# noorgme/Decentralised-Verification-and-Distributed-Execution-of-Large-Scale-Video-Diffusion-Models

Measured on AMD Instinct MI355X. Metric: denoising steps/sec, Zeroscope-XL 24f@1024x576 (CFG UNet3D forward + guidance + DDIM), higher is better.
Workload: dtype f16

## Files before the change

### decentralised-verification-and-distributed-execution-of-large-scale-video-diffusion-models_amd/_lib.py

```python
from __future__ import annotations

import ctypes as C
import os

_HERE = os.path.dirname(os.path.abspath(__file__))
LIB_PATH = os.environ.get("VDX_LIB_PATH") or os.path.join(_HERE, "libvdx_hip.so")


class GemmArgs(C.Structure):
    _fields_ = [
        ("a", C.c_void_p), ("a2", C.c_void_p), ("w", C.c_void_p), ("bias", C.c_void_p),
        ("bias2", C.c_void_p), ("residual", C.c_void_p), ("out", C.c_void_p),
        ("M", C.c_int32), ("N", C.c_int32), ("K", C.c_int32), ("mode", C.c_int32),
        ("c1", C.c_int32), ("c2", C.c_int32),
        ("lda", C.c_int32), ("lda2", C.c_int32), ("ldo", C.c_int32), ("ldr", C.c_int32),
        ("h_in", C.c_int32), ("w_in", C.c_int32), ("h_out", C.c_int32), ("w_out", C.c_int32),
        ("stride", C.c_int32), ("upsample", C.c_int32), ("frames", C.c_int32), ("hw", C.c_int32),
        ("rows_per_bias2", C.c_int32), ("ldb2", C.c_int32), ("epilogue", C.c_int32),
        ("row_begin", C.c_int32), ("row_end", C.c_int32),
        ("ksplit", C.c_int32), ("wset_rows", C.c_int32), ("workspace", C.c_void_p), ("wset_bias", C.c_void_p),
        ("workspace_bytes", C.c_size_t), ("pad_mode", C.c_int32),
    ]


class ClipPreprocessArgs(C.Structure):
    _fields_ = [
        ("frames", C.c_void_p), ("x_bounds", C.c_void_p), ("x_coeffs", C.c_void_p), ("y_bounds", C.c_void_p),
        ("y_coeffs", C.c_void_p), ("out", C.c_void_p), ("out_u8", C.c_void_p),
        ("frame_pitch", C.c_size_t), ("row_pitch", C.c_int32), ("F", C.c_int32), ("H", C.c_int32), ("W", C.c_int32),
        ("kx", C.c_int32), ("ky", C.c_int32), ("band", C.c_int32), ("span", C.c_int32), ("ldo", C.c_int32),
    ]


_vp, _i, _f, _sz = C.c_void_p, C.c_int, C.c_float, C.c_size_t

SIGNATURES = {
    "vdx_last_error": (C.c_char_p, []),
    "vdx_version": (_i, []),
    "vdx_build_flags": (_i, []),
    "vdx_gemm_f16": (_i, [C.POINTER(GemmArgs), _vp]),
    "vdx_gemm_plan": (_i, [C.POINTER(GemmArgs), C.POINTER(C.c_int32), C.POINTER(C.c_int32)]),
    "vdx_gemm_kernel_name": (_i, [C.POINTER(GemmArgs), C.c_char_p, _sz]),
    "vdx_gemm_plan_ksplit": (_i, [C.POINTER(GemmArgs), C.POINTER(C.c_int32), C.POINTER(C.c_int32), C.POINTER(C.c_size_t)]),
    "vdx_softmax_rows_f16": (_i, [_vp, _i, _i, _i, _f, _vp]),
    "vdx_rows_to_u8_frames": (_i, [_vp, _i, _sz, _vp, _vp]),
    "vdx_im2col_in_f16": (_i, [_vp, _vp, _i, _i, _i, _i, _i, _i, _vp]),
    "vdx_rows_to_ncfhw_f16": (_i, [_vp, _i, _vp, _i, _i, _i, _i, _i, _vp]),
    "vdx_silu_f16": (_i, [_vp, _vp, _sz, _vp]),
    "vdx_groupnorm_workspace": (_sz, [_i, _i, _i, _i]),
    "vdx_groupnorm_f16": (_i, [_vp, _i, _i, _vp, _i, _i, _vp, _vp, _f, _i, _i, _i, _i, _vp, _i, _vp, _vp]),
    "vdx_groupnorm_workspace_part": (_sz, [_i, _i, _i, _i, _i]),
    "vdx_groupnorm_part_f16": (_i, [_vp, _i, _i, _vp, _i, _i, _vp, _vp, _f, _i, _i, _i, _i, _vp, _i, _vp, _i, _vp]),
    "vdx_groupnorm_fold_linear_f16": (_i, [_vp, _i, _i, _vp, _vp, _f, _i, _i, _i, _vp, _i, _vp, _vp, _i, _vp, _vp, _vp]),
    "vdx_groupnorm_stats_f16": (_i, [_vp, _i, _i, _vp, _i, _i, _vp, _vp, _f, _i, _i, _i, _vp, _i, C.POINTER(_sz), _vp]),
    "vdx_conv3x3_gn_supported": (_i, [_i, _i, _i]),
    "vdx_conv3x3_gn_preferred": (_i, [_i, _i, _i, _i, _i, _i]),
    "vdx_conv3x3_gn_f16": (_i, [_vp, _i, _vp, _i, _i, _i, _vp, _vp, _vp, _vp, _i, _i, _vp, _i, _vp, _i, _i, _i, _i, _i, _vp]),
    "vdx_tconv_gn_supported": (_i, [_i, _i, _i]),
    "vdx_tconv_gn_preferred": (_i, [_i, _i, _i, _i, _i]),
    "vdx_tconv_gn_f16": (_i, [_vp, _i, _vp, _vp, _vp, _vp, _i, _vp, _i, _i, _i, _i, _i, _i, _vp]),
    "vdx_layernorm_f16": (_i, [_vp, _i, _vp, _vp, _f, _i, _i, _vp, _i, _vp]),
    "vdx_flash_attn_f16": (_i, [_vp, _i, _vp, _i, _vp, _i, _vp, _i, _i, _i, _i, _i, _i, _i, _f, _i, _vp]),
    "vdx_flash_attn_rows_f16": (_i, [_vp, _i, _vp, _i, _vp, _i, _vp, _i, _i, _i, _i, _i, _i, _i, _f, _i, _vp]),
    "vdx_timestep_embedding_f16": (_i, [_vp, _vp, _i, _i, _vp]),
    "vdx_gelu_f16": (_i, [_vp, _vp, _sz, _vp]),
    "vdx_temporal_attn_f16": (_i, [_vp, _i, _vp, _i, _i, _i, _i, _i, _f, _vp]),
    "vdx_ff_block_supported": (_i, [_i]),
    "vdx_ff_block_pack_bytes": (_sz, [_i]),
    "vdx_ff_block_f16": (_i, [_vp, _i, _vp, _f, _vp, _i, _i, _i, _vp]),
    "vdx_ff_block_proj_pack_bytes": (_sz, [_i]),
    "vdx_ff_block_proj_f16": (_i, [_vp, _i, _vp, _f, _vp, _i, _i, _vp, _vp, _i, _i, _i, _vp]),
    "vdx_cross_attn_block_supported": (_i, [_i, _i]),
    "vdx_cross_attn_block_pack_bytes": (_sz, [_i]),
    "vdx_cross_attn_block_kv_bytes": (_sz, [_i]),
    "vdx_cross_attn_block_f16": (_i, [_vp, _i, _vp, _vp, _i, _f, _vp, _i, _i, _i, _i, _vp]),
    "vdx_temporal_attn_block_supported": (_i, [_i, _i]),
    "vdx_temporal_attn_block_wqkv_bytes": (_sz, [_i]),
    "vdx_temporal_attn_block_wo_bytes": (_sz, [_i]),
    "vdx_temporal_attn_block_f16": (_i, [_vp, _i, _vp, _vp, _f, _vp, _vp, _vp, _vp, _i, _i, _i, _i, _i, _f, _vp]),
    "vdx_temporal_attn_block2_supported": (_i, [_i, _i]),
    "vdx_temporal_attn_block2_pack_bytes": (_sz, [_i]),
    "vdx_temporal_attn_block2_f16": (_i, [_vp, _i, _vp, _f, _vp, _i, _i, _i, _i, _i, _vp]),
    "vdx_comm_unique_id": (_i, [_vp]),
    "vdx_comm_init": (_i, [_vp, _i, _i, C.POINTER(_vp)]),
    "vdx_comm_destroy": (_i, [_vp]),
    "vdx_allgather_shard": (_i, [_vp, _vp, _vp, _sz, _vp]),
    "vdx_halo_exchange": (_i, [_vp, _vp, _sz, _i, _vp, _sz, _i, _vp]),
    "vdx_ipc_export": (_i, [_vp, _vp, C.POINTER(_sz)]),
    "vdx_ipc_open": (_i, [_vp, _sz, C.POINTER(_vp)]),
    "vdx_ipc_close": (_i, [_vp, _sz]),
# ... 84 lines not shown
```

### decentralised-verification-and-distributed-execution-of-large-scale-video-diffusion-models_amd/ops.py

```python
from __future__ import annotations

import contextlib
import ctypes as C
from typing import Optional

import torch

from . import _lib
from ._lib import GemmArgs, VdxError

PLAIN, CONV3X3, TCONV3 = 0, 1, 2
EPI_GEGLU = 1


def _stream() -> int:
    return torch.cuda.current_stream().cuda_stream


def _p(t: Optional[torch.Tensor], name: str, dtype=torch.float16) -> Optional[int]:
    if t is None:
        return None
    if not t.is_cuda:
        raise VdxError(f"{name}: expected a GPU tensor (the denoising path has no CPU fallback)")
    if t.dtype != dtype:
# ... 423 lines not shown
def conv3x3_gn(x, gamma, beta, w, *, x2=None, bias=None, bias2=None, rows_per_bias2=0, residual=None, groups, n_img, h, wd, eps,
               partition_samples=0, out=None):
    r, c1, ldx = _rows(x, "x")
    S = h * wd
    M = n_img * S
    c2 = ldx2 = 0
    if x2 is not None:
        r2, c2, ldx2 = _rows(x2, "x2")
        if r2 < M:
            raise VdxError(f"conv3x3_gn: x2 has {r2} rows, need {M}")
    Cc = c1 + c2
    N, K = w.shape
    if r < M or K != 9 * Cc or gamma.numel() != Cc or beta.numel() != Cc or not w.is_contiguous():
        raise VdxError(f"conv3x3_gn: x [{r}][{c1}] (+{c2}), w [{N}][{K}], gamma {gamma.numel()}, M = {M}: shapes do not match")
    if not conv3x3_gn_supported(c1, c2, N):
        raise VdxError(f"conv3x3_gn: c1={c1}, c2={c2}, N={N} not supported")
    if bias is not None and bias.numel() != N:
        raise VdxError(f"conv3x3_gn: bias has {bias.numel()} elements, N={N}")
    ldb2 = _covers(bias2, M, N, "conv3x3_gn", "bias2", rows_per_bias2)
    ldr = _covers(residual, M, N, "conv3x3_gn", "residual")
    out, ldo = _out(out, M, N, x, "conv3x3_gn")
    need = _lib.load().vdx_groupnorm_workspace_part(n_img, S, Cc, groups, partition_samples)
    ws = _scratch(_GN_WS, x.device, need, torch.uint8, 1 << 20)
    off = C.c_size_t(0)
    _launch("vdx_groupnorm_stats_f16", _p(x, "x"), c1, ldx, _p(x2, "x2"), c2, ldx2, _p(gamma, "gamma"), _p(beta, "beta"),
            float(eps), groups, n_img, S, ws.data_ptr(), partition_samples, C.byref(off))
    with _timed("conv3x3_gn_kernel", 2.0 * M * N * K, (M, N, K)):
        _launch("vdx_conv3x3_gn_f16", _p(x, "x"), ldx, _p(x2, "x2"), ldx2, c1, c2, ws.data_ptr() + off.value, _p(w, "w"),
                _p(bias, "bias"), _p(bias2, "bias2"), rows_per_bias2, ldb2, _p(residual, "residual"), ldr, _p(out, "out"), ldo,
                n_img, h, wd, N)
    return out


def tconv_gn_supported(C: int, N: int, F: int) -> bool:
    return bool(_lib.load().vdx_tconv_gn_supported(C, N, F))


def tconv_gn_preferred(C: int, N: int, B: int, F: int, S: int) -> bool:
    return bool(_lib.load().vdx_tconv_gn_preferred(C, N, B, F, S))


def tconv_gn(x, gamma, beta, w, *, bias=None, residual=None, groups, B, F, S, eps, partition_samples=0, out=None):
    r, Cc, ldx = _rows(x, "x")
    M = B * F * S
    N, K = w.shape
    if r < M or K != 3 * Cc or gamma.numel() != Cc or beta.numel() != Cc or not w.is_contiguous():
        raise VdxError(f"tconv_gn: x [{r}][{Cc}], w [{N}][{K}], gamma {gamma.numel()}, M = {M}: shapes do not match")
    if not tconv_gn_supported(Cc, N, F):
        raise VdxError(f"tconv_gn: C={Cc}, N={N}, F={F} not supported")
    if bias is not None and bias.numel() != N:
        raise VdxError(f"tconv_gn: bias has {bias.numel()} elements, N={N}")
    ldr = _covers(residual, M, N, "tconv_gn", "residual")
    out, ldo = _out(out, M, N, x, "tconv_gn")
    need = _lib.load().vdx_groupnorm_workspace_part(B, F * S, Cc, groups, partition_samples)
    ws = _scratch(_GN_WS, x.device, need, torch.uint8, 1 << 20)
    off = C.c_size_t(0)
    _launch("vdx_groupnorm_stats_f16", _p(x, "x"), Cc, ldx, None, 0, 0, _p(gamma, "gamma"), _p(beta, "beta"), float(eps), groups, B,
            F * S, ws.data_ptr(), partition_samples, C.byref(off))
    with _timed(f"tconv_gn_kernel<{16 if F % 16 == 0 else 12 if F % 12 == 0 else 8}>", 2.0 * M * N * K, (M, N, K)):
        _launch("vdx_tconv_gn_f16", _p(x, "x"), ldx, ws.data_ptr() + off.value, _p(w, "w"), _p(bias, "bias"),
                _p(residual, "residual"), ldr, _p(out, "out"), ldo, B, F, S, Cc, N)
    return out


def layernorm(x, gamma, beta, *, M, eps=1e-5, out=None):
    r, Cc, ldx = _rows(x, "x")
# ... 511 lines not shown
```

### decentralised-verification-and-distributed-execution-of-large-scale-video-diffusion-models_amd/unet3d.py

```python
from __future__ import annotations

import math
import os
from dataclasses import dataclass
from types import SimpleNamespace
from typing import Dict, List, Optional, Tuple

import torch
import torch.nn as nn

from . import ops, packing
from ._lib import VdxError


@dataclass
class UNet3DConfig:
    in_channels: int = 4
    out_channels: int = 4
    block_out_channels: Tuple[int, ...] = (320, 640, 1280, 1280)
    layers_per_block: int = 2
    attention_head_dim: int = 64
    cross_attention_dim: int = 1024
    norm_num_groups: int = 32
    norm_eps: float = 1e-5
# ... 9 lines not shown


TEXT_PAD = 128


class UNet3DConditionModel(nn.Module):

    def __init__(self, cfg: Optional[UNet3DConfig] = None):
        super().__init__()
        self.cfg = cfg or UNet3DConfig.zeroscope()
        c = self.cfg
        if c.attention_head_dim != 64:
            raise VdxError("attention kernels are built for head_dim 64")
        for ch in c.block_out_channels:
            if ch % 64 != 0:
                raise VdxError("block_out_channels must be multiples of 64")
        if c.cross_attention_dim % 64 != 0:
            raise VdxError("cross_attention_dim must be a multiple of 64")
        self.config = SimpleNamespace(in_channels=c.in_channels, out_channels=c.out_channels,
                                      cross_attention_dim=c.cross_attention_dim,
                                      block_out_channels=c.block_out_channels,
                                      sample_size=None)
        self.W: Dict[str, torch.Tensor] = {}
        self._temb_slices: Dict[str, Tuple[int, int]] = {}
        self._device = torch.device("cpu")
        self.dtype = torch.float16
        self.ff_block_bytes = None
        self.lean_concat = True
        self.lean_attn = True
        self.fold_norm_proj_in = True
        self.fuse_ff = True
        self.fuse_cross_attn = True
        self.fuse_proj_out = True
        self.fuse_conv_gn = True
        self.fuse_tconv = True
        self.spatial_v_rows = True
        self.fuse_temporal_attention = True
        self.share_cfg_prefix = True
        self.detect_cfg_duplicate = False
        self._text_ref = None
        self._text_kv: Dict[str, tuple] = {}

    def _resnet_names(self) -> List[str]:
        c = self.cfg
        names = []
        for i, t in enumerate(c.down_block_types):
            names += [f"down_blocks.{i}.resnets.{j}" for j in range(c.layers_per_block)]
        names += ["mid_block.resnets.0", "mid_block.resnets.1"]
        for i, t in enumerate(c.up_block_types):
            names += [f"up_blocks.{i}.resnets.{j}" for j in range(c.layers_per_block + 1)]
        return names

    @torch.no_grad()
    def load_diffusers_state_dict(self, sd: Dict[str, torch.Tensor], device=None):
        dev = torch.device(device) if device is not None else self._device
        W: Dict[str, torch.Tensor] = {}

        def put(name, t):
            W[name] = t.to(device=dev, dtype=torch.float16).contiguous()

        used = set()

        def get(k):
            used.add(k)
            if k not in sd:
                raise VdxError(f"missing key in state dict: {k}")
# ... 496 lines not shown
        x = self._temp_conv("mid_block.temp_convs.0", x, B, F, hh * ww)
        x = self._spatial_transformer("mid_block.attentions.0", x, ehs_pad, n_img, F, hh, ww)
        x = self._temporal_transformer("mid_block.temp_attentions.0", x, B, F, hh * ww, x.shape[1] // 64)
        x = self._resnet("mid_block.resnets.1", x, None, temb_all, n_img, F, hh, ww)
        x = self._temp_conv("mid_block.temp_convs.1", x, B, F, hh * ww)
        for i, t in enumerate(c.up_block_types):
            p = f"up_blocks.{i}"
            for j in range(c.layers_per_block + 1):
                skip, sh, sw = skips.pop()
                if (sh, sw) != (hh, ww):
                    raise VdxError("skip connection resolution mismatch")
                if shared_skip and not skips:
                    skip = torch.cat([skip, skip])
                owned = [x, skip]
                x = skip = None
                x = self._resnet(f"{p}.resnets.{j}", owned, None, temb_all, n_img, F, hh, ww)
                x = self._temp_conv(f"{p}.temp_convs.{j}", x, B, F, hh * ww)
                if t.startswith("CrossAttn"):
                    x = self._spatial_transformer(f"{p}.attentions.{j}", x, ehs_pad, n_img, F, hh, ww)
                    x = self._temporal_transformer(f"{p}.temp_attentions.{j}", x, B, F, hh * ww, x.shape[1] // 64)
            if i != nlev - 1:
                th, tw = skips[-1][1], skips[-1][2]
                w_up = W[f"{p}.upsamplers.0.conv.weight"]
                if (th, tw) == (2 * hh, 2 * ww):
                    mode_up = 3
                elif hh <= th <= 2 * hh and ww <= tw <= 2 * ww:
                    mode_up = 2
                    w_up = W[f"{p}.upsamplers.0.conv.weight_taps9"]
                else:
                    raise VdxError(f"upsampler {p}: {hh}x{ww} -> {th}x{tw}")
                x = ops.gemm(x, w_up, M=n_img * th * tw, mode=ops.CONV3X3,
                             bias=W[f"{p}.upsamplers.0.conv.bias"], conv=(n_img, hh, ww, th, tw, 1, mode_up), allow_ksplit=True)
                hh, ww = th, tw
        n = ops.groupnorm(x, W["conv_norm_out.weight"], W["conv_norm_out.bias"], groups=c.norm_num_groups,
                          n_samples=n_img, rows_per_sample=hh * ww, eps=c.norm_eps, silu_act=True)
        y = ops.gemm(n, W["conv_out.weight"], M=n_img * hh * ww, mode=ops.CONV3X3, bias=W["conv_out.bias"],
                     conv=(n_img, hh, ww, hh, ww, 1, False))
        out = ops.rows_to_ncfhw(y, B, c.out_channels, F, hh, ww)
        return SimpleNamespace(sample=out)
```

### include/vdx.h

```cpp
#ifndef VDX_H
#define VDX_H
#include <stddef.h>
#include <stdint.h>

#ifdef __cplusplus
extern "C" {
#endif

typedef void* vdx_stream_t;

const char* vdx_last_error(void);
int vdx_version(void);
int vdx_build_flags(void);

enum { VDX_GEMM_PLAIN = 0, VDX_GEMM_CONV3X3 = 1, VDX_GEMM_TCONV3 = 2 };
enum { VDX_EPI_GEGLU = 1 };

typedef struct vdx_gemm_args {
    const void* a;
    const void* a2;
    const void* w;
    const void* bias;
    const void* bias2;
    const void* residual;
// ... 28 lines not shown
                      int Kpad, vdx_stream_t stream);

int vdx_rows_to_ncfhw_f16(const void* rows, int ld, void* out, int B, int C, int F, int H, int W,
                          vdx_stream_t stream);

int vdx_silu_f16(const void* x, void* y, size_t n, vdx_stream_t stream);

int vdx_timestep_embedding_f16(const float* t_device, void* out, int B, int dim, vdx_stream_t stream);

int vdx_gelu_f16(const void* x, void* y, size_t n, vdx_stream_t stream);

size_t vdx_groupnorm_workspace(int n_samples, int rows_per_sample, int C, int G);
int vdx_groupnorm_f16(const void* x, int c1, int ldx, const void* x2, int c2, int ldx2,
                      const void* gamma, const void* beta, float eps, int G,
                      int n_samples, int rows_per_sample, int silu,
                      void* y, int ldy, void* workspace, vdx_stream_t stream);
size_t vdx_groupnorm_workspace_part(int n_samples, int rows_per_sample, int C, int G, int partition_samples);
int vdx_groupnorm_fold_linear_f16(const void* x, int C, int ldx, const void* gamma, const void* beta, float eps, int G,
                                  int n_samples, int rows_per_sample, void* workspace, int partition_samples,
                                  const void* w, const void* bias, int N, void* w_out, void* bias_out, vdx_stream_t stream);
int vdx_groupnorm_part_f16(const void* x, int c1, int ldx, const void* x2, int c2, int ldx2,
                           const void* gamma, const void* beta, float eps, int G,
                           int n_samples, int rows_per_sample, int silu,
                           void* y, int ldy, void* workspace, int partition_samples, vdx_stream_t stream);
int vdx_groupnorm_stats_f16(const void* x, int c1, int ldx, const void* x2, int c2, int ldx2, const void* gamma,
                            const void* beta, float eps, int G, int n_samples, int rows_per_sample, void* workspace,
                            int partition_samples, size_t* scale_shift_offset, vdx_stream_t stream);
int vdx_conv3x3_gn_supported(int c1, int c2, int N);
int vdx_conv3x3_gn_preferred(int c1, int c2, int N, int n_img, int h, int w);
int vdx_conv3x3_gn_f16(const void* a, int lda, const void* a2, int lda2, int c1, int c2, const float* scale_shift,
                       const void* w, const void* bias, const void* bias2, int rows_per_bias2, int ldb2,
                       const void* residual, int ldr, void* out, int ldo, int n_img, int h, int w_px, int N,
                       vdx_stream_t stream);
int vdx_tconv_gn_supported(int C, int N, int F);
int vdx_tconv_gn_preferred(int C, int N, int B, int F, int S);
int vdx_tconv_gn_f16(const void* x, int ldx, const float* scale_shift, const void* w, const void* bias,
                     const void* residual, int ldr, void* out, int ldo, int B, int F, int S, int C, int N,
                     vdx_stream_t stream);
int vdx_softmax_rows_f16(void* x, int ld, int rows, int cols, float scale, vdx_stream_t stream);

int vdx_layernorm_f16(const void* x, int ldx, const void* gamma, const void* beta, float eps,
                      int M, int C, void* y, int ldy, vdx_stream_t stream);

int vdx_flash_attn_f16(const void* q, int ldq, const void* k, int ldk, const void* vt, int ldvt,
                       void* out, int ldo, int n_seq, int sq, int skv, int skv_pad, int heads,
                       int seq_per_kv, float scale, int causal, vdx_stream_t stream);
int vdx_flash_attn_rows_f16(const void* q, int ldq, const void* k, int ldk, const void* v, int ldv,
                            void* out, int ldo, int n_seq, int sq, int skv, int skv_pad, int heads,
                            int seq_per_kv, float scale, int causal, vdx_stream_t stream);

int vdx_ff_block_supported(int inner);
size_t vdx_ff_block_pack_bytes(int inner);
int vdx_ff_block_f16(const void* t, int ldt, const void* packed, float eps, void* out, int ldo, int M, int inner,
                     vdx_stream_t stream);
size_t vdx_ff_block_proj_pack_bytes(int inner);
int vdx_ff_block_proj_f16(const void* t, int ldt, const void* packed, float eps, const void* x, int ldx, int xrows,
                          const void* proj_packed, void* out, int ldo, int M, int inner, vdx_stream_t stream);

int vdx_temporal_attn_f16(const void* qkv, int ldqkv, void* out, int ldo, int B, int F, int HW,
                          int heads, float scale, vdx_stream_t stream);

int vdx_temporal_attn_block_supported(int inner, int F);
size_t vdx_temporal_attn_block_wqkv_bytes(int inner);
size_t vdx_temporal_attn_block_wo_bytes(int inner);
int vdx_temporal_attn_block_f16(const void* t, int ldt, const void* gamma, const void* beta, float eps,
                                const void* wqkv_packed, const void* wo_packed, const void* bo,
// ... 124 lines not shown
```

### decentralised-verification-and-distributed-execution-of-large-scale-video-diffusion-models_amd/csrc/gemm_ws.hip

```cpp
#include "gemm_common.h"
#include "lab.h"

#ifdef VDX_STAMPS
VDX_STAMP_BUFFER(g_ws_stamps, vdx_debug_read_ws_stamps, 256 * 4)
#define WS_T() __builtin_amdgcn_s_memtime()
#endif

namespace {

template <int N>
__device__ __forceinline__ void wait_vmcnt() {
    asm volatile("s_waitcnt vmcnt(%0)" ::"n"(N) : "memory");
}

struct WsP {
    GemmP g;
    int nt;
    int groups;
    int nch;
    int per_xcd;
};

template <int K, int NW, int ROWS, bool GEGLU, bool RES, bool PIPE, bool WSET = false>
struct Ws {
    static constexpr int KS = K / 32;
    static constexpr int MT = ROWS / 16;
    static constexpr int SUBT = ROWS * 128;
    static constexpr int STAGE = ROWS * K * 2;
#ifdef VDX_WS_NS3
    static constexpr int NS = 3;
#else
    static constexpr int NS = (K == 640 && 4 * STAGE + (GEGLU ? GELU_TAB_BYTES : 0) + (WSET ? NW * 64 * 32 : 0) <= 160 * 1024) ? 4 : 3;
#endif
    static constexpr int PF = NS - 1;
    static constexpr int PPW = STAGE / 1024 / NW;
    static constexpr int RB = ROWS / 8;
    static_assert(PPW * NW * 1024 == STAGE, "chunk must split evenly over the waves");
    static_assert(NS * STAGE <= 160 * 1024, "ring exceeds the LDS");
    typedef f32x4 Acc[MT][2];

    const GemmP& p;
    char* smem;
    const float2* gelu;
    int lane, wave, frow, fq, n0, c0, nch;
    bool active;
    const f16* a_src;
    f16x8 wf[KS][2];
    f16x8 bv;
    int set_left;
    int cur_set;
#ifdef VDX_STAMPS
    unsigned long long t_bar = 0, t_iss = 0, t_wait = 0, t_last = 0;
#endif

    __device__ __forceinline__ Ws(const GemmP& p_, char* smem_) : p(p_), smem(smem_) {}

    __device__ __forceinline__ void issue(int k) {
        const f16* src = a_src + (size_t)(c0 + k) * ROWS * p.lda;
        char* dst = smem + (k % NS) * STAGE;
#pragma unroll
        for (int i = 0; i < PPW; ++i) {
            const int piece = wave * PPW + i, q = piece / RB, rb = piece % RB;
            __builtin_amdgcn_global_load_lds((gptr_t)(src + (size_t)(8 * rb) * p.lda + 64 * q),
                                             (lptr_t)(dst + q * SUBT + rb * 1024), 16, 0, 0);
        }
    }
    template <int N>
    __device__ __forceinline__ void wait_le(int n) {
        if constexpr (N == 0) wait_vmcnt<0>();
        else {
            if (n >= N) wait_vmcnt<N>();
            else wait_le<N - 1>(n);
        }
    }
    __device__ __forceinline__ void sync(int k) {
        constexpr int LAG = PIPE ? 1 : 0;
        int nd = 0, ns = 0;
#pragma unroll
        for (int j = 1; j < PF; ++j) nd += (k + j < nch);
#pragma unroll
        for (int j = 1; j <= PF; ++j) ns += (active && k >= j + LAG);
        int nr = 0;
        if (RES && PIPE) {
#pragma unroll
            for (int j = 1; j <= PF; ++j) nr += (active && k >= j);
        }
        wait_le<(PF - 1) * PPW + PF * MT * ((RES && PIPE) ? 2 : 1)>(__builtin_amdgcn_readfirstlane(nd * PPW + (ns + nr) * MT));
#ifdef VDX_STAMPS
        const unsigned long long t0 = WS_T();
#endif
        __builtin_amdgcn_s_barrier();
#ifdef VDX_STAMPS
        const unsigned long long t1 = WS_T();
#endif
        if (k + PF < nch) issue(k + PF);
#ifdef VDX_STAMPS
        const unsigned long long t2 = WS_T();
        t_bar += t1 - t0;
        t_iss += t2 - t1;
        t_wait += t0 - t_last;
        t_last = t2;
#endif
    }
    __device__ __forceinline__ void zero(Acc& acc) {
#pragma unroll
        for (int i = 0; i < MT; ++i) acc[i][0] = acc[i][1] = (f32x4){0.f, 0.f, 0.f, 0.f};
    }
    __device__ __forceinline__ void load_af(const char* st, int s, f16x8 (&af)[MT]) {
        const int c = (s & 1) * 4 + fq;
#pragma unroll
        for (int i = 0; i < MT; ++i)
            af[i] = *(const f16x8*)(st + (s >> 1) * SUBT + i * 2048 + ((c ^ (frow & 7)) << 4));
    }
    __device__ __forceinline__ void mfma_step(int s, const f16x8 (&af)[MT], Acc& acc) {
        f32x4 z0 = (f32x4){0.f, 0.f, 0.f, 0.f}, z1 = z0;
        if (WSET && s == 0) {
            int o = bias_off();
            asm volatile("" : "+v"(o));
            z0 = *(const f32x4*)(smem + o);
            z1 = *(const f32x4*)(smem + o + 16);
        }
#pragma unroll
        for (int i = 0; i < MT; ++i) {
            acc[i][0] = __builtin_amdgcn_mfma_f32_16x16x32_f16(wf[s][0], af[i], s == 0 ? z0 : acc[i][0], 0, 0, 0);
            acc[i][1] = __builtin_amdgcn_mfma_f32_16x16x32_f16(wf[s][1], af[i], s == 0 ? z1 : acc[i][1], 0, 0, 0);
        }
    }
    __device__ __forceinline__ int bias_off() const { return NS * STAGE + (int)threadIdx.x * 32; }
    __device__ __forceinline__ void load_weights(int set) {
        const int nw = active ? n0 : 0;
        const f16* wbase = p.w + (WSET ? (size_t)set * p.N * K : 0);
#pragma unroll
        for (int j = 0; j < 2; ++j) {
            const f16* wrow = wbase + (size_t)(nw + 8 * (frow >> 2) + 4 * j + (frow & 3)) * K + 8 * fq;
#pragma unroll
            for (int s = 0; s < KS; ++s) wf[s][j] = *(const f16x8*)(wrow + 32 * s);
        }
        if (WSET) {
            const float* b = p.wset_bias + (size_t)set * p.N + nw + 8 * fq;
            *(f32x4*)(smem + bias_off()) = *(const f32x4*)b;
            *(f32x4*)(smem + bias_off() + 16) = *(const f32x4*)(b + 4);
        }
    }
    __device__ __forceinline__ void load_res(int k, f16x8 (&rv)[MT]) {
        const size_t m = (size_t)(c0 + k) * ROWS + frow;
#pragma unroll
        for (int i = 0; i < MT; ++i) rv[i] = *(const f16x8*)(p.res + (m + 16 * i) * p.ldr + n0 + 8 * fq);
    }
    __device__ __forceinline__ void store_group(int k, int i, const Acc& acc, const f16x8 (&rv)[MT]) {
        const size_t m = (size_t)(c0 + k) * ROWS + frow + 16 * i;
        float v[8];
#pragma unroll
        for (int j = 0; j < 4; ++j) {
            v[j] = acc[i][0][j] + (float)bv[j];
            v[4 + j] = acc[i][1][j] + (float)bv[4 + j];
        }
        if (GEGLU) {
            f16x4 o;
#pragma unroll
            for (int j = 0; j < 4; ++j) o[j] = (f16)(v[j] * gelu_tab(v[4 + j], gelu));
            *(f16x4*)(p.out + m * p.ldo + ((n0 + 8 * fq) >> 1)) = o;
        } else {
            f16x8 o;
#pragma unroll
            for (int j = 0; j < 8; ++j) o[j] = (f16)(RES ? v[j] + (float)rv[i][j] : v[j]);
            *(f16x8*)(p.out + m * p.ldo + n0 + 8 * fq) = o;
        }
    }
    typedef f16x8 Res[MT];
    template <bool HAS_PREV>
    __device__ __forceinline__ void step(int k, Acc& cur, const Acc& prev, Res& rv_next, const Res& rv) {
        const char* st = smem + (k % NS) * STAGE + frow * 128;
        if (!active) zero(cur);
        if (!active) return;
        if (RES && PIPE) load_res(k, rv_next);
        if (WSET) {
            if (set_left == 0) {
                cur_set += 1;
                set_left = p.wset_rows / ROWS;
                load_weights(cur_set);
            }
            set_left -= 1;
        }
#pragma unroll
        for (int s = 0; s < KS; ++s) {
            f16x8 af[MT];
            load_af(st, s, af);
            mfma_step(s, af, cur);
            if (HAS_PREV) {
#pragma unroll
                for (int i = 0; i < MT; ++i)
                    if (s + 1 == KS * (i + 1) / MT) store_group(k - 1, i, prev, rv);
            }
        }
    }
    __device__ __forceinline__ void drain(int k, const Acc& acc, Res& rv) {
        if (!active) return;
        if (RES && !PIPE) load_res(k, rv);
#pragma unroll
        for (int i = 0; i < MT; ++i) store_group(k, i, acc, rv);
    }

    __device__ __forceinline__ void run(const WsP& q) {
        const int tid = threadIdx.x;
        gelu = (const float2*)(smem + NS * STAGE);
        if (GEGLU) gelu_tab_init((float2*)(smem + NS * STAGE), tid, NW * 64);
        lane = tid & 63;
        wave = __builtin_amdgcn_readfirstlane(tid >> 6);
        frow = lane & 15;
        fq = lane >> 4;
        const int slot = (blockIdx.x & 7) * q.per_xcd + (blockIdx.x >> 3);
        const int group = slot / q.nt, panel = slot - group * q.nt;
        if (group >= q.groups) return;
        c0 = (int)((long long)q.nch * group / q.groups);
        nch = (int)((long long)q.nch * (group + 1) / q.groups) - c0;
        if (nch <= 0) return;
        n0 = panel * (32 * NW) + wave * 32;
        active = n0 < p.N;
        a_src = p.a + (size_t)(lane >> 3) * p.lda + ((lane & 7) ^ (lane >> 3)) * 8;
#pragma unroll
        for (int j = 0; j < PF; ++j)
            if (j < nch) issue(j);
#ifdef VDX_STAMPS
        t_last = WS_T();
#endif

        cur_set = 0;
        set_left = 0;
        if (WSET) {
            const int cps = p.wset_rows / ROWS;
            cur_set = c0 / cps;
            set_left = cps - (c0 - cur_set * cps);
        }
        load_weights(cur_set);
#pragma unroll
        for (int j = 0; j < 8; ++j) bv[j] = (f16)0.f;
        if (p.bias && active) bv = *(const f16x8*)(p.bias + n0 + 8 * fq);

        Res r0, r1;
#pragma unroll
        for (int i = 0; i < MT; ++i) r0[i] = r1[i] = bv;
        if (!PIPE) {
            for (int k = 0; k < nch; ++k) {
                sync(k);
                Acc acc;
                step<false>(k, acc, acc, r0, r0);
                drain(k, acc, r0);
            }
        } else {
            Acc a, b;
            sync(0);
            step<false>(0, a, a, r0, r1);
            int k = 1;
            for (; k + 1 < nch; k += 2) {
                sync(k);
                step<true>(k, b, a, r1, r0);
                sync(k + 1);
                step<true>(k + 1, a, b, r0, r1);
            }
            if (k < nch) {
                sync(k);
                step<true>(k, b, a, r1, r0);
                drain(k, b, r1);
            } else {
                drain(nch - 1, a, r0);
            }
        }
#ifdef VDX_STAMPS
        if (threadIdx.x == 0) {
            unsigned long long* d = g_ws_stamps + blockIdx.x * 4;
            d[0] = t_bar; d[1] = t_iss; d[2] = t_wait; d[3] = (unsigned long long)nch;
        }
#endif
    }
};

template <int K, int NW, int ROWS, bool GEGLU, bool RES, bool PIPE, bool WSET>
__global__ __launch_bounds__(NW * 64) void gemm_ws_kernel(const WsP q) {
    extern __shared__ __attribute__((aligned(16))) char smem[];
    Ws<K, NW, ROWS, GEGLU, RES, PIPE, WSET> ws(q.g, smem);
    ws.run(q);
}

template <int K, int NW, int ROWS, bool GEGLU, bool RES, bool PIPE, bool WSET = false>
int launch_ws(const GemmP& p, const GemmSink& to) {
    if (to.name)
        return snprintf(to.name, GEMM_NAME_MAX, "gemm_ws_kernel<%d, %d, %d, %s, %s, %s, %s>", K, NW, ROWS, tf(GEGLU), tf(RES), tf(PIPE), tf(WSET)), 0;
    typedef Ws<K, NW, ROWS, GEGLU, RES, PIPE, WSET> W;
    static_assert(!(WSET && GEGLU), "weight sets run the plain epilogue");
    constexpr int lds = W::NS * W::STAGE + (GEGLU ? GELU_TAB_BYTES : 0) + (WSET ? NW * 64 * 32 : 0);
    auto kern = gemm_ws_kernel<K, NW, ROWS, GEGLU, RES, PIPE, WSET>;
    static const hipError_t attr_rc = hipFuncSetAttribute((const void*)kern, hipFuncAttributeMaxDynamicSharedMemorySize, lds);
    if (attr_rc != hipSuccess) return vdx_fail("gemm_ws: cannot reserve %d bytes of LDS", lds);
    WsP q;
    q.g = p;
// ... 49 lines not shown
```

Before: 6.183.

## Fuse final GroupNorm+SiLU, conv_out and NCFHW layout into one kernel

Adds a dedicated kernel for the UNet's final output stage. It applies GroupNorm scale/shift and SiLU on the fly, runs a 3x3 conv to 4 channels using MFMA with a per-tap partial-sum ring buffer over row strips, and writes NCFHW directly. This removes the separate normalized activation tensor, a poorly shaped N=4 GEMM and the layout conversion pass at full 128x72 resolution. The cost is a specialised kernel limited to C=320, four output channels and W<=256, which adds complexity and correctness risk around strip boundaries.

```diff
diff --git a/decentralised-verification-and-distributed-execution-of-large-scale-video-diffusion-models_amd/_lib.py b/decentralised-verification-and-distributed-execution-of-large-scale-video-diffusion-models_amd/_lib.py
--- a/decentralised-verification-and-distributed-execution-of-large-scale-video-diffusion-models_amd/_lib.py
+++ b/decentralised-verification-and-distributed-execution-of-large-scale-video-diffusion-models_amd/_lib.py
@@ -56,6 +56,8 @@
     "vdx_conv3x3_gn_supported": (_i, [_i, _i, _i]),
     "vdx_conv3x3_gn_preferred": (_i, [_i, _i, _i, _i, _i, _i]),
     "vdx_conv3x3_gn_f16": (_i, [_vp, _i, _vp, _i, _i, _i, _vp, _vp, _vp, _vp, _i, _i, _vp, _i, _vp, _i, _i, _i, _i, _i, _vp]),
+    "vdx_conv_out_gn_supported": (_i, [_i, _i, _i, _i]),
+    "vdx_conv_out_gn_f16": (_i, [_vp, _i, _vp, _vp, _vp, _vp, _i, _i, _i, _i, _i, _i, _i, _vp]),
     "vdx_tconv_gn_supported": (_i, [_i, _i, _i]),
     "vdx_tconv_gn_preferred": (_i, [_i, _i, _i, _i, _i]),
     "vdx_tconv_gn_f16": (_i, [_vp, _i, _vp, _vp, _vp, _vp, _i, _vp, _i, _i, _i, _i, _i, _i, _vp]),
diff --git a/decentralised-verification-and-distributed-execution-of-large-scale-video-diffusion-models_amd/csrc/conv_out.hip b/decentralised-verification-and-distributed-execution-of-large-scale-video-diffusion-models_amd/csrc/conv_out.hip
--- /dev/null
+++ b/decentralised-verification-and-distributed-execution-of-large-scale-video-diffusion-models_amd/csrc/conv_out.hip
@@ -0,0 +1,146 @@
+#include "vdx_common.h"
+
+typedef float f32x2 __attribute__((ext_vector_type(2)));
+
+constexpr int CO_PX = 64;
+constexpr int CO_THREADS = 256;
+constexpr int CO_MAX_W = 256;
+
+static int co_ring(int W) {
+    int r = 128;
+    while (r < 2 * W + 2 + CO_PX) r <<= 1;
+    return r;
+}
+
+template <int KS>
+__global__ __launch_bounds__(CO_THREADS) void conv_out_gn_kernel(const f16* __restrict__ x, int ldx, const float* __restrict__ ab,
+                                                                 const f16* __restrict__ w, const f16* __restrict__ bias,
+                                                                 f16* __restrict__ out, int F, int H, int W, int strip_rows,
+                                                                 int strips, int ring_mask) {
+    constexpr int C = 32 * KS;
+    extern __shared__ f32x4 co_lds[];
+    float* abl = (float*)co_lds;
+    f32x4* P = co_lds + C / 2;
+    f32x4* ring = P + CO_PX * 9;
+    const int tid = threadIdx.x, lane = tid & 63, wave = tid >> 6, j = lane & 15, q = lane >> 4;
+    const int img = blockIdx.x / strips, strip = blockIdx.x - img * strips;
+    const int S = H * W;
+    const int y0 = strip * strip_rows, y1 = min(H, y0 + strip_rows);
+    const int in_begin = max(0, y0 - 1) * W, in_end = min(H, y1 + 1) * W;
+    const int o_begin = y0 * W, o_end = y1 * W;
+
+    for (int i = tid * 4; i < 2 * C; i += 4 * CO_THREADS) {
+        const f32x4 t = *(const f32x4*)(ab + (size_t)img * C * 2 + i);
+        *(f32x4*)(abl + i) = (f32x4){t[0], t[2], t[1], t[3]};
+    }
+    f16x8 wf[3][KS];
+#pragma unroll
+    for (int t = 0; t < 3; ++t) {
+        const int n = 16 * t + j;
+#pragma unroll
+        for (int s = 0; s < KS; ++s) {
+            const int c = 32 * s + 8 * q;
+            wf[t][s] = (f16x8){0, 0, 0, 0, 0, 0, 0, 0};
+            if (n < 36) wf[t][s] = *(const f16x8*)(w + (size_t)(n & 3) * 9 * C + (c >> 6) * 576 + (n >> 2) * 64 + (c & 63));
+        }
+    }
+    const f32x4 bias4 = {(float)bias[0], (float)bias[1], (float)bias[2], (float)bias[3]};
+    const f16* xi = x + (size_t)img * S * ldx + 8 * q;
+    auto load = [&](int cs, f16x8(&xr)[KS]) __attribute__((always_inline)) {
+        const int px = min(cs + wave * 16 + j, in_end - 1);
+        const f16* src = xi + (size_t)px * ldx;
+#pragma unroll
+        for (int s = 0; s < KS; ++s) xr[s] = *(const f16x8*)(src + 32 * s);
+    };
+    auto silu8 = [&](const f16x8 v, const f32x4(&t)[4]) __attribute__((always_inline)) {
+        f16x8 o;
+#pragma unroll
+        for (int k = 0; k < 4; ++k) {
+            const f32x2 xv = {(float)v[2 * k], (float)v[2 * k + 1]};
+            const f32x2 y = xv * (f32x2){t[k][0], t[k][1]} + (f32x2){t[k][2], t[k][3]};
+            const f32x2 u = y * -1.44269504088896341f;
+            const f32x2 d = (f32x2){__builtin_amdgcn_exp2f(u[0]), __builtin_amdgcn_exp2f(u[1])} + 1.0f;
+            const f32x2 r = y * (f32x2){__builtin_amdgcn_rcpf(d[0]), __builtin_amdgcn_rcpf(d[1])};
+            o[2 * k] = (f16)r[0];
+            o[2 * k + 1] = (f16)r[1];
+        }
+        return o;
+    };
+
+    f16x8 xr[KS], xn[KS];
+    load(in_begin, xr);
+    __syncthreads();
+    for (int cs = in_begin; cs < in_end; cs += CO_PX) {
+        const int ce = min(cs + CO_PX, in_end);
+        const bool more = cs + CO_PX < in_end;
+        if (more) load(cs + CO_PX, xn);
+        f32x4 acc[3];
+#pragma unroll
+        for (int t = 0; t < 3; ++t) acc[t] = (f32x4){0.f, 0.f, 0.f, 0.f};
+#pragma unroll
+        for (int s = 0; s < KS; ++s) {
+            const float* a = abl + (32 * s + 8 * q) * 2;
+            const f32x4 t4[4] = {*(const f32x4*)a, *(const f32x4*)(a + 4), *(const f32x4*)(a + 8), *(const f32x4*)(a + 12)};
+            const f16x8 nv = silu8(xr[s], t4);
+#pragma unroll
+            for (int t = 0; t < 3; ++t) acc[t] = __builtin_amdgcn_mfma_f32_16x16x32_f16(wf[t][s], nv, acc[t], 0, 0, 0);
+        }
+        f32x4* pp = P + (wave * 16 + j) * 9;
+        pp[q] = acc[0];
+        pp[4 + q] = acc[1];
+        if (q == 0) pp[8] = acc[2];
+        __syncthreads();
+        const bool first_chunk = cs == in_begin, last_chunk = ce == in_end;
+        const int lo = max(o_begin, cs - W - 1), hi = min(o_end, ce + W + 1);
+        for (int p = lo + tid; p < hi; p += CO_THREADS) {
+            const int y = p / W, xx = p - y * W;
+            f32x4 a4 = (first_chunk || p >= cs + W + 1) ? bias4 : ring[p & ring_mask];
+#pragma unroll
+            for (int ky = 0; ky < 3; ++ky)
+#pragma unroll
+                for (int kx = 0; kx < 3; ++kx) {
+                    const int src = p + (ky - 1) * W + (kx - 1);
+                    const bool in_img = (unsigned)(y + ky - 1) < (unsigned)H && (unsigned)(xx + kx - 1) < (unsigned)W;
+                    if (in_img && src >= cs && src < ce) a4 += P[(src - cs) * 9 + ky * 3 + kx];
+                }
+            if (last_chunk || p + W + 1 < ce) {
+                const int b = img / F, f = img - b * F;
+#pragma unroll
+                for (int o = 0; o < 4; ++o) out[((size_t)(b * 4 + o) * F + f) * S + p] = (f16)a4[o];
+            } else {
+                ring[p & ring_mask] = a4;
+            }
+        }
+        __syncthreads();
+        if (more) {
+#pragma unroll
+            for (int s = 0; s < KS; ++s) xr[s] = xn[s];
+        }
+    }
+}
+
+extern "C" int vdx_conv_out_gn_supported(int C, int out_ch, int H, int W) {
+    return C == 320 && out_ch == 4 && H > 0 && W > 0 && W <= CO_MAX_W && (long long)H * W < (1ll << 30) ? 1 : 0;
+}
+
+extern "C" int vdx_conv_out_gn_f16(const void* x, int ldx, const float* scale_shift, const void* w, const void* bias, void* out,
+                                   int B, int F, int H, int W, int C, int out_ch, int strip_rows, vdx_stream_t stream) {
+    VDX_CHECK(x && scale_shift && w && bias && out, "conv_out_gn: null pointer");
+    VDX_CHECK(vdx_conv_out_gn_supported(C, out_ch, H, W), "conv_out_gn: C=%d, out_ch=%d, %dx%d not supported (C = 320, 4 channels, W <= %d)",
+              C, out_ch, H, W, CO_MAX_W);
+    VDX_CHECK(B > 0 && F > 0 && strip_rows >= 0, "conv_out_gn: bad B=%d F=%d strip_rows=%d", B, F, strip_rows);
+    VDX_CHECK(ldx % 8 == 0 && ldx >= C, "conv_out_gn: ldx=%d must be a multiple of 8 >= C", ldx);
+    VDX_CHECK((uintptr_t)x % 16 == 0 && (uintptr_t)scale_shift % 16 == 0 && (uintptr_t)w % 16 == 0, "conv_out_gn: pointers must be 16-byte aligned");
+    const long long n_img = (long long)B * F;
+    int rows = strip_rows > 0 ? strip_rows : 8;
+    if (strip_rows == 0)
+        while (rows < H && n_img * ((H + rows - 1) / rows) > 2ll * vdx_num_cus()) ++rows;
+    if (rows > H) rows = H;
+    const int strips = (H + rows - 1) / rows;
+    VDX_CHECK(n_img * strips < (1ll << 31), "conv_out_gn: too many strips");
+    const int ring = co_ring(W);
+    const size_t lds = ((size_t)C / 2 + CO_PX * 9 + ring) * sizeof(f32x4);
+    hipLaunchKernelGGL(conv_out_gn_kernel<10>, dim3((unsigned)(n_img * strips)), dim3(CO_THREADS), lds, (hipStream_t)stream,
+                       (const f16*)x, ldx, scale_shift, (const f16*)w, (const f16*)bias, (f16*)out, F, H, W, rows, strips, ring - 1);
+    return vdx_launch_status("vdx_conv_out_gn_f16");
+}
diff --git a/decentralised-verification-and-distributed-execution-of-large-scale-video-diffusion-models_amd/ops.py b/decentralised-verification-and-distributed-execution-of-large-scale-video-diffusion-models_amd/ops.py
--- a/decentralised-verification-and-distributed-execution-of-large-scale-video-diffusion-models_amd/ops.py
+++ b/decentralised-verification-and-distributed-execution-of-large-scale-video-diffusion-models_amd/ops.py
@@ -479,6 +479,35 @@
     return out
 
 
+def conv_out_gn_supported(C: int, out_ch: int, H: int, W: int) -> bool:
+    return bool(_lib.load().vdx_conv_out_gn_supported(C, out_ch, H, W))
+
+
+def conv_out_gn(x, gamma, beta, w, bias, *, groups, B, F, H, W, out_ch, eps, strip_rows=0, out=None):
+    r, Cc, ldx = _rows(x, "x")
+    n_img, S = B * F, H * W
+    M = n_img * S
+    if r < M or w.dim() != 2 or w.shape[0] < out_ch or w.shape[1] != 9 * Cc or not w.is_contiguous() or bias.numel() < out_ch \
+            or gamma.numel() != Cc or beta.numel() != Cc:
+        raise VdxError(f"conv_out_gn: x [{r}][{Cc}], w {tuple(w.shape)}, bias {bias.numel()}, gamma {gamma.numel()}, M = {M}: "
+                       "shapes do not match")
+    if not conv_out_gn_supported(Cc, out_ch, H, W):
+        raise VdxError(f"conv_out_gn: C={Cc}, out_ch={out_ch}, {H}x{W} not supported")
+    if out is None:
+        out = torch.empty((B, out_ch, F, H, W), dtype=torch.float16, device=x.device)
+    if tuple(out.shape) != (B, out_ch, F, H, W) or not out.is_contiguous():
+        raise VdxError("conv_out_gn: bad out")
+    need = _lib.load().vdx_groupnorm_workspace_part(n_img, S, Cc, groups, 0)
+    ws = _scratch(_GN_WS, x.device, need, torch.uint8, 1 << 20)
+    off = C.c_size_t(0)
+    _launch("vdx_groupnorm_stats_f16", _p(x, "x"), Cc, ldx, None, 0, 0, _p(gamma, "gamma"), _p(beta, "beta"), float(eps), groups,
+            n_img, S, ws.data_ptr(), 0, C.byref(off))
+    with _timed("conv_out_gn_kernel", 2.0 * M * out_ch * 9 * Cc, (M, out_ch, 9 * Cc)):
+        _launch("vdx_conv_out_gn_f16", _p(x, "x"), ldx, ws.data_ptr() + off.value, _p(w, "w"), _p(bias, "bias"), _p(out, "out"),
+                B, F, H, W, Cc, out_ch, int(strip_rows))
+    return out
+
+
 def tconv_gn_supported(C: int, N: int, F: int) -> bool:
     return bool(_lib.load().vdx_tconv_gn_supported(C, N, F))
 
diff --git a/decentralised-verification-and-distributed-execution-of-large-scale-video-diffusion-models_amd/unet3d.py b/decentralised-verification-and-distributed-execution-of-large-scale-video-diffusion-models_amd/unet3d.py
--- a/decentralised-verification-and-distributed-execution-of-large-scale-video-diffusion-models_amd/unet3d.py
+++ b/decentralised-verification-and-distributed-execution-of-large-scale-video-diffusion-models_amd/unet3d.py
@@ -65,6 +65,7 @@
         self.fuse_ff = True
         self.fuse_cross_attn = True
         self.fuse_proj_out = True
+        self.fuse_conv_out = True
         self.fuse_conv_gn = True
         self.fuse_tconv = True
         self.spatial_v_rows = True
@@ -627,6 +628,10 @@
                 x = ops.gemm(x, w_up, M=n_img * th * tw, mode=ops.CONV3X3,
                              bias=W[f"{p}.upsamplers.0.conv.bias"], conv=(n_img, hh, ww, th, tw, 1, mode_up), allow_ksplit=True)
                 hh, ww = th, tw
+        if self.fuse_conv_out and ops.conv_out_gn_supported(x.shape[1], c.out_channels, hh, ww):
+            out = ops.conv_out_gn(x, W["conv_norm_out.weight"], W["conv_norm_out.bias"], W["conv_out.weight"], W["conv_out.bias"],
+                                  groups=c.norm_num_groups, B=B, F=F, H=hh, W=ww, out_ch=c.out_channels, eps=c.norm_eps)
+            return SimpleNamespace(sample=out)
         n = ops.groupnorm(x, W["conv_norm_out.weight"], W["conv_norm_out.bias"], groups=c.norm_num_groups,
                           n_samples=n_img, rows_per_sample=hh * ww, eps=c.norm_eps, silu_act=True)
         y = ops.gemm(n, W["conv_out.weight"], M=n_img * hh * ww, mode=ops.CONV3X3, bias=W["conv_out.bias"],
diff --git a/include/vdx.h b/include/vdx.h
--- a/include/vdx.h
+++ b/include/vdx.h
@@ -84,6 +84,9 @@
                        const void* w, const void* bias, const void* bias2, int rows_per_bias2, int ldb2,
                        const void* residual, int ldr, void* out, int ldo, int n_img, int h, int w_px, int N,
                        vdx_stream_t stream);
+int vdx_conv_out_gn_supported(int C, int out_ch, int H, int W);
+int vdx_conv_out_gn_f16(const void* x, int ldx, const float* scale_shift, const void* w, const void* bias, void* out,
+                        int B, int F, int H, int W, int C, int out_ch, int strip_rows, vdx_stream_t stream);
 int vdx_tconv_gn_supported(int C, int N, int F);
 int vdx_tconv_gn_preferred(int C, int N, int B, int F, int S);
 int vdx_tconv_gn_f16(const void* x, int ldx, const float* scale_shift, const void* w, const void* bias,
```

Measured after the change: 6.198 (median of 6 runs). No clear change (+0.2%).

## Split residual GEMM pipeline into steady-state and tail loops with exact vmcnt waits

Applied to the files above, without the earlier changes.

For the residual-fused pipelined GEMM path, the main loop is split into a steady-state phase that always issues the next prefetch and tail phases that issue none. This lets the vmcnt wait use a tighter compile-time range. Residual loads become inline-asm global loads whose completion is tied to exact vmcnt waits placed just before the first store that needs them, with scheduling fences after each issue. The aim is to stop the compiler from inserting conservative full waits that serialise residual loads with the LDS prefetch. In exchange, the hand-counted vmcnt values are fragile and a wrong count would read residuals before they land.

```diff
diff --git a/decentralised-verification-and-distributed-execution-of-large-scale-video-diffusion-models_amd/csrc/gemm_ws.hip b/decentralised-verification-and-distributed-execution-of-large-scale-video-diffusion-models_amd/csrc/gemm_ws.hip
--- a/decentralised-verification-and-distributed-execution-of-large-scale-video-diffusion-models_amd/csrc/gemm_ws.hip
+++ b/decentralised-verification-and-distributed-execution-of-large-scale-video-diffusion-models_amd/csrc/gemm_ws.hip
@@ -37,6 +37,7 @@
     static constexpr int RB = ROWS / 8;
     static_assert(PPW * NW * 1024 == STAGE, "chunk must split evenly over the waves");
     static_assert(NS * STAGE <= 160 * 1024, "ring exceeds the LDS");
+    static constexpr int WAIT_MAX = (PF - 1) * PPW + PF * MT * ((RES && PIPE) ? 2 : 1);
     typedef f32x4 Acc[MT][2];
 
     const GemmP& p;
@@ -65,19 +66,27 @@
                                              (lptr_t)(dst + q * SUBT + rb * 1024), 16, 0, 0);
         }
     }
-    template <int N>
+    template <int N, int LO = 0>
     __device__ __forceinline__ void wait_le(int n) {
-        if constexpr (N == 0) wait_vmcnt<0>();
+        if constexpr (N == LO) wait_vmcnt<LO>();
         else {
             if (n >= N) wait_vmcnt<N>();
-            else wait_le<N - 1>(n);
-        }
-    }
+            else wait_le<N - 1, LO>(n);
+        }
+    }
+    enum { ISSUE_NONE, ISSUE_ALWAYS, ISSUE_IF };
+    __device__ __forceinline__ void fence() {
+        asm volatile("" ::: "memory");
+        __builtin_amdgcn_sched_barrier(0);
+    }
+    template <int ISSUE>
     __device__ __forceinline__ void sync(int k) {
         constexpr int LAG = PIPE ? 1 : 0;
-        int nd = 0, ns = 0;
-#pragma unroll
-        for (int j = 1; j < PF; ++j) nd += (k + j < nch);
+        int nd = ISSUE == ISSUE_ALWAYS ? PF - 1 : 0, ns = 0;
+        if (ISSUE != ISSUE_ALWAYS) {
+#pragma unroll
+            for (int j = 1; j < PF; ++j) nd += (k + j < nch);
+        }
 #pragma unroll
         for (int j = 1; j <= PF; ++j) ns += (active && k >= j + LAG);
         int nr = 0;
@@ -85,7 +94,7 @@
 #pragma unroll
             for (int j = 1; j <= PF; ++j) nr += (active && k >= j);
         }
-        wait_le<(PF - 1) * PPW + PF * MT * ((RES && PIPE) ? 2 : 1)>(__builtin_amdgcn_readfirstlane(nd * PPW + (ns + nr) * MT));
+        wait_le<WAIT_MAX, ISSUE == ISSUE_ALWAYS ? (PF - 1) * PPW : 0>(__builtin_amdgcn_readfirstlane(nd * PPW + (ns + nr) * MT));
 #ifdef VDX_STAMPS
         const unsigned long long t0 = WS_T();
 #endif
@@ -93,7 +102,8 @@
 #ifdef VDX_STAMPS
         const unsigned long long t1 = WS_T();
 #endif
-        if (k + PF < nch) issue(k + PF);
+        if (ISSUE == ISSUE_ALWAYS || (ISSUE == ISSUE_IF && k + PF < nch)) issue(k + PF);
+        if (RES && PIPE) fence();
 #ifdef VDX_STAMPS
         const unsigned long long t2 = WS_T();
         t_bar += t1 - t0;
@@ -145,7 +155,16 @@
     __device__ __forceinline__ void load_res(int k, f16x8 (&rv)[MT]) {
         const size_t m = (size_t)(c0 + k) * ROWS + frow;
 #pragma unroll
-        for (int i = 0; i < MT; ++i) rv[i] = *(const f16x8*)(p.res + (m + 16 * i) * p.ldr + n0 + 8 * fq);
+        for (int i = 0; i < MT; ++i) {
+            const f16* src = p.res + (m + 16 * i) * p.ldr + n0 + 8 * fq;
+            asm volatile("global_load_dwordx4 %0, %1, off" : "=v"(rv[i]) : "v"(src) : "memory");
+        }
+    }
+    template <int N>
+    __device__ __forceinline__ void res_landed(f16x8 (&rv)[MT]) {
+        static_assert(MT == 2 || MT == 4, "one operand per residual register set");
+        if constexpr (MT == 2) asm volatile("s_waitcnt vmcnt(%2)" : "+v"(rv[0]), "+v"(rv[1]) : "n"(N) : "memory");
+        else asm volatile("s_waitcnt vmcnt(%4)" : "+v"(rv[0]), "+v"(rv[1]), "+v"(rv[2]), "+v"(rv[3]) : "n"(N) : "memory");
     }
     __device__ __forceinline__ void store_group(int k, int i, const Acc& acc, const f16x8 (&rv)[MT]) {
         const size_t m = (size_t)(c0 + k) * ROWS + frow + 16 * i;
@@ -168,8 +187,8 @@
         }
     }
     typedef f16x8 Res[MT];
-    template <bool HAS_PREV>
-    __device__ __forceinline__ void step(int k, Acc& cur, const Acc& prev, Res& rv_next, const Res& rv) {
+    template <bool HAS_PREV, int ISSUE, bool ST2 = false>
+    __device__ __forceinline__ void step(int k, Acc& cur, const Acc& prev, Res& rv_next, Res& rv) {
         const char* st = smem + (k % NS) * STAGE + frow * 128;
         if (!active) zero(cur);
         if (!active) return;
@@ -190,13 +209,28 @@
             if (HAS_PREV) {
 #pragma unroll
                 for (int i = 0; i < MT; ++i)
-                    if (s + 1 == KS * (i + 1) / MT) store_group(k - 1, i, prev, rv);
-            }
+                    if (s + 1 == KS * (i + 1) / MT) {
+                        if (RES && i == 0) res_landed<(ST2 ? MT : 0) + (ISSUE == ISSUE_ALWAYS ? PPW : 0) + MT>(rv);
+                        store_group(k - 1, i, prev, rv);
+                    }
+            }
+        }
+    }
+    __device__ __forceinline__ void hand_over(Acc& a, Res& ra, const Acc& b, Res& rb) {
+        if (active) res_landed<MT>(rb);
+#pragma unroll
+        for (int i = 0; i < MT; ++i) {
+            a[i][0] = b[i][0];
+            a[i][1] = b[i][1];
+            ra[i] = rb[i];
         }
     }
     __device__ __forceinline__ void drain(int k, const Acc& acc, Res& rv) {
         if (!active) return;
-        if (RES && !PIPE) load_res(k, rv);
+        if (RES && !PIPE) {
+            load_res(k, rv);
+            res_landed<0>(rv);
+        }
 #pragma unroll
         for (int i = 0; i < MT; ++i) store_group(k, i, acc, rv);
     }
@@ -242,25 +276,56 @@
         for (int i = 0; i < MT; ++i) r0[i] = r1[i] = bv;
         if (!PIPE) {
             for (int k = 0; k < nch; ++k) {
-                sync(k);
+                sync<ISSUE_IF>(k);
                 Acc acc;
-                step<false>(k, acc, acc, r0, r0);
+                step<false, ISSUE_IF>(k, acc, acc, r0, r0);
                 drain(k, acc, r0);
             }
+        } else if (RES) {
+            Acc a, b;
+            sync<ISSUE_IF>(0);
+            step<false, ISSUE_IF>(0, a, a, r0, r1);
+            if (nch == 1) res_landed<0>(r0);
+            int k = 1;
+            if (k + 1 + PF < nch) {
+                sync<ISSUE_ALWAYS>(1);
+                step<true, ISSUE_ALWAYS, false>(1, b, a, r1, r0);
+                sync<ISSUE_ALWAYS>(2);
+                step<true, ISSUE_ALWAYS, true>(2, a, b, r0, r1);
+                k = 3;
+            }
+            for (; k + 1 + PF < nch; k += 2) {
+                sync<ISSUE_ALWAYS>(k);
+                step<true, ISSUE_ALWAYS, true>(k, b, a, r1, r0);
+                sync<ISSUE_ALWAYS>(k + 1);
+                step<true, ISSUE_ALWAYS, true>(k + 1, a, b, r0, r1);
+            }
+            if (k + PF < nch) {
+                sync<ISSUE_ALWAYS>(k);
+                step<true, ISSUE_ALWAYS>(k, b, a, r1, r0);
+                hand_over(a, r0, b, r1);
+                k += 1;
+            }
+            for (; k < nch; ++k) {
+                sync<ISSUE_NONE>(k);
+                step<true, ISSUE_NONE>(k, b, a, r1, r0);
+                hand_over(a, r0, b, r1);
+            }
+            drain(nch - 1, a, r0);
         } else {
             Acc a, b;
-            sync(0);
-            step<false>(0, a, a, r0, r1);
+            sync<ISSUE_IF>(0);
+            step<false, ISSUE_IF>(0, a, a, r0, r1);
             int k = 1;
             for (; k + 1 < nch; k += 2) {
-                sync(k);
-                step<true>(k, b, a, r1, r0);
-                sync(k + 1);
-                step<true>(k + 1, a, b, r0, r1);
+                sync<ISSUE_IF>(k);
+                step<true, ISSUE_IF>(k, b, a, r1, r0);
+                sync<ISSUE_IF>(k + 1);
+                step<true, ISSUE_IF>(k + 1, a, b, r0, r1);
             }
             if (k < nch) {
-                sync(k);
-                step<true>(k, b, a, r1, r0);
+                sync<ISSUE_IF>(k);
+                step<true, ISSUE_IF>(k, b, a, r1, r0);
                 drain(k, b, r1);
             } else {
                 drain(nch - 1, a, r0);
```

Result: no change. 6.121 before, 6.127 after (median of 6 runs) (+0.1%).
